# Audio-WestlakeU/FN-SSL

Measured on AMD Instinct MI355X. Metric: TF-frames/sec DP-IPD forward, 4-mic 257-bin x 300-frame, higher is better.
Workload: dtype f32; 1 GPU; BASELINE configs[1]: FN-SSL (online) DP-IPD forward, waveform->STFT->features->3x(full-band BiLSTM + narrow-band LSTM)->head; 32 utterances/GPU x 4 mics ('MM' = 6 pairs) x 257 bins x 300 frames, fp32; frame = one STFT frame of one utterance; stream_chunk_frames=0, utterances_per_gpu=32, global_batch=32, mics=4, pairs_per_utterance=6, frames=300, bins=257, parallelism=dp1 (utterance shards, no collective), chunk_pairs=0

## Files before the change

fn-ssl_amd/csrc/forward.hip:

```cpp
#include <algorithm>

#include "common.h"

namespace {

size_t align_up(size_t v, size_t a) { return (v + a - 1) / a * a; }

struct Plan {
  int chunk;
  size_t act_floats;
  size_t lstm_ws;
  size_t head_floats;
  size_t total;
};

Plan make_plan(int nb, int nf, int nt, int is_online, int chunk_pairs) {
  Plan p;
  p.chunk = (chunk_pairs <= 0 || chunk_pairs > nb) ? nb : chunk_pairs;
  p.act_floats = (size_t)p.chunk * nt * nf * 256;
  const size_t ws_full = fnssl_lstm_workspace_bytes_ex(p.chunk * nt, 128, 2, FNSSL_PRECISION_FP32);
  const size_t ws_narr = is_online ? fnssl_lstm_workspace_bytes_ex(p.chunk * nf, 256, 1, FNSSL_PRECISION_FP32)
                                   : fnssl_lstm_workspace_bytes_ex(p.chunk * nf, 128, 2, FNSSL_PRECISION_FP32);
  p.lstm_ws = align_up(std::max(ws_full, ws_narr), 256);
  p.head_floats = (size_t)p.chunk * (nt / FNSSL_SEG_FRAMES) * 2 * nf;
  p.total = 6 * align_up(p.act_floats * 4, 256) + p.lstm_ws + align_up(p.head_floats * 4, 256) + 256;
  return p;
}

}

extern "C" {

size_t fnssl_forward_workspace_bytes(int nb, int nf, int nt, int is_online, int chunk_pairs) {
  if (nb <= 0 || nf <= 0 || nt <= 0) return 0;
  return make_plan(nb, nf, nt, is_online, chunk_pairs).total;
}

int fnssl_forward(const fnssl_net* net, const float* x0, int nb, int nf, int nt, float* out, void* workspace,
                  size_t workspace_bytes, int chunk_pairs, void* stream) {
  FNSSL_REQUIRE(net && x0, "forward: null pointer");
  FNSSL_REQUIRE(nb > 0 && nf > 0 && nt > 0, "forward: empty problem (nb %d, nf %d, nt %d)", nb, nf, nt);
  if (nt / FNSSL_SEG_FRAMES == 0) return FNSSL_OK;
  FNSSL_REQUIRE(out, "forward: null output pointer");
  FNSSL_REQUIRE(net->input_size > 0 && net->input_size % 4 == 0, "forward: input_size %d must be a multiple of 4",
                net->input_size);
  FNSSL_REQUIRE(!net->doa_wt || nf == 256, "forward: the DOA layer needs nf = 256 (Linear(512, 180))");
  const Plan pl = make_plan(nb, nf, nt, net->is_online, chunk_pairs);
  if (!workspace || workspace_bytes < pl.total) {
    fnssl::set_error("forward: workspace %zu < %zu bytes", workspace_bytes, pl.total);
    return FNSSL_E_WORKSPACE;
  }
  char* wsb = static_cast<char*>(workspace);
  wsb = reinterpret_cast<char*>(align_up(reinterpret_cast<uintptr_t>(wsb), 256));
  const size_t act_bytes = align_up(pl.act_floats * 4, 256);
  float* F[2] = {reinterpret_cast<float*>(wsb), reinterpret_cast<float*>(wsb + act_bytes)};
  float* N[2] = {reinterpret_cast<float*>(wsb + 2 * act_bytes), reinterpret_cast<float*>(wsb + 3 * act_bytes)};
  float* Sf = reinterpret_cast<float*>(wsb + 4 * act_bytes);
  float* Sn = reinterpret_cast<float*>(wsb + 5 * act_bytes);
  float* lws = reinterpret_cast<float*>(wsb + 6 * act_bytes);
  float* head_tmp = reinterpret_cast<float*>(wsb + 6 * act_bytes + pl.lstm_ws);

  const int cin = net->input_size;
  const int nt2 = nt / FNSSL_SEG_FRAMES;
  const int narr_h = net->is_online ? 256 : 128;
  const int narr_dirs = net->is_online ? 1 : 2;
  const long long C = 256;
  const long long PS = (long long)nt * nf * C;
  const fnssl_view fl_by_full = {nullptr, PS, (long long)nf * C, C};
  const fnssl_view fl_by_narr = {nullptr, PS, C, (long long)nf * C};
  const fnssl_view nl_by_full = {nullptr, PS, C, (long long)nt * C};
  const fnssl_view nl_by_narr = {nullptr, PS, (long long)nt * C, C};
  auto with = [](fnssl_view v, const float* p) {
    v.p = p;
    return v;
  };

  for (int p0 = 0; p0 < nb; p0 += pl.chunk) {
    const int G = std::min(pl.chunk, nb - p0);
    const float* xc = x0 + (size_t)p0 * nt * nf * cin;
    for (int blk = 0; blk < 3; ++blk) {
      float* Fo = F[blk & 1];
      float* No = N[blk & 1];
      const float* Np = N[(blk + 1) & 1];
      fnssl_lstm_desc d = {};
      d.hidden = 128;
      d.ndir = 2;
      d.nseq = G * nt;
      d.q_inner = nt;
      d.nsteps = nf;
      if (blk == 0) {
        d.src0 = fnssl_view{xc, (long long)nt * nf * cin, (long long)nf * cin, cin};
        d.c0 = cin;
      } else {
        d.src0 = with(nl_by_full, Sn);
        d.c0 = 256;
      }
      d.out = Fo;
      d.out_so = fl_by_full.so;
      d.out_si = fl_by_full.si;
      d.out_st = fl_by_full.st;
      if (blk > 0) {
        d.skip = with(nl_by_full, Np);
        d.out_sum = Sf;
      }
      d.wpack[0] = net->wpack[blk][0][0];
      d.wpack[1] = net->wpack[blk][0][1];
      d.workspace = lws;
      d.workspace_bytes = pl.lstm_ws;
      d.fallback_count = net->fallback_count;
      d.tuning = net->tuning;
      int rc = fnssl_lstm_forward(&d, stream);
      if (rc != FNSSL_OK) return rc;
      fnssl_lstm_desc e = {};
      e.hidden = narr_h;
      e.ndir = narr_dirs;
      e.nseq = G * nf;
      e.q_inner = nf;
      e.nsteps = nt;
      e.c0 = 256;
      if (blk == 0) {
        e.src0 = with(fl_by_narr, Fo);
        e.src2 = fnssl_view{xc, (long long)nt * nf * cin, cin, (long long)nf * cin};
        e.c2 = cin;
      } else {
        e.src0 = with(fl_by_narr, Sf);
      }
      e.out = No;
      e.out_so = nl_by_narr.so;
      e.out_si = nl_by_narr.si;
      e.out_st = nl_by_narr.st;
      if (blk < 2) {
        e.skip = with(fl_by_narr, Fo);
        e.out_sum = Sn;
      }
      e.wpack[0] = net->wpack[blk][1][0];
      e.wpack[1] = net->wpack[blk][1][1];
      e.workspace = lws;
      e.workspace_bytes = pl.lstm_ws;
      e.fallback_count = net->fallback_count;
      e.tuning = net->tuning;
      rc = fnssl_lstm_forward(&e, stream);
      if (rc != FNSSL_OK) return rc;
    }
    if (nt2 > 0) {
      if (net->doa_wt) {
        int rc = fnssl_head(N[0], G, nf, nt, net->emb_w, net->emb_b, head_tmp, stream);
        if (rc != FNSSL_OK) return rc;
        rc = fnssl_linear(head_tmp, G * nt2, 2 * nf, net->doa_wt, net->doa_b, 180,
                          out + (size_t)p0 * nt2 * 180, stream);
        if (rc != FNSSL_OK) return rc;
      } else {
        int rc = fnssl_head(N[0], G, nf, nt, net->emb_w, net->emb_b, out + (size_t)p0 * nt2 * 2 * nf, stream);
        if (rc != FNSSL_OK) return rc;
      }
    }
  }
  return FNSSL_OK;
}

}
```

fn-ssl_amd/csrc/lstm.hip:

```cpp
#include <algorithm>
#include <cstdlib>
#include <cstring>
#include <vector>

#include "common.h"
#include "tuning.h"

#include "lstm_static.h"
#include "lstm_bf16.h"
#include "lstm_bf16w.h"
#include "lstm_split_static.h"

using namespace fnssl_lstm;

namespace fnssl_lstm {
extern template int launch_h<16>(int, const LstmParams&, int, int, const LaunchCtx&);
extern template int launch_h<32>(int, const LstmParams&, int, int, const LaunchCtx&);
extern template int launch_h<64>(int, const LstmParams&, int, int, const LaunchCtx&);
extern template int launch_h<128>(int, const LstmParams&, int, int, const LaunchCtx&);
extern template int launch_h<256>(int, const LstmParams&, int, int, const LaunchCtx&);
extern template int launch_split_h<128>(int, const LstmParams&, int, int, const LaunchCtx&);
extern template int launch_split_h<256>(int, const LstmParams&, int, int, const LaunchCtx&);
int forward_save(LstmParams p, int H, int mode, const LaunchCtx& lc);
int forward_bf16(LstmParams p, int H, const LaunchCtx& lc);
// ... 232 lines not shown
}

static LstmParams fwd_params(const fnssl_lstm_desc* d, const LstmWsLayout& ws) {
  LstmParams p;
  p.src0 = View{d->src0.p, d->src0.so, d->src0.si, d->src0.st};
  p.src1 = View{d->src1.p, d->src1.so, d->src1.si, d->src1.st};
  p.src2 = View{d->src2.p, d->src2.so, d->src2.si, d->src2.st};
  p.skip = View{d->skip.p, d->skip.so, d->skip.si, d->skip.st};
  p.carry = d->carry_state ? 1 : 0;
  p.out = d->carry_state ? d->out - d->out_st : d->out;
  p.out_sum = (d->carry_state && d->out_sum) ? d->out_sum - d->out_st : d->out_sum;
  p.out_so = d->out_so;
  p.out_si = d->out_si;
  p.out_st = d->out_st;
  p.wpack[0] = d->wpack[0];
  p.wpack[1] = d->wpack[1];
  p.cscratch = d->workspace;
  p.cluster_ws = reinterpret_cast<char*>(d->workspace) + ws.cluster.off;
  p.reserve = d->reserve;
  p.ntasks = (d->nseq + 15) / 16;
  p.c0 = d->c0;
  p.c2 = d->c2;
  p.nseq = d->nseq;
  p.q_inner = d->q_inner;
  p.nsteps = d->nsteps;
  p.ndir = d->ndir;
  p.quads_per_slice = quads_per_slice(d->c0, d->c2, d->hidden);
#ifdef FNSSL_BUILD_ABLATE
  p.ablate = env_int("FNSSL_ABLATE", 1, 255);
#else
  p.ablate = 0;
#endif
  p.fallback_count = d->fallback_count;
  return p;
}

struct Fp32Call {
  const fnssl_lstm_desc* d;
  const LstmWsLayout& ws;
  const LaunchCtx& lc;
  LstmParams p;
  int H, mode;
  int* family;
  int* rounds;
  int nlaunch = 0;
  void report(int f) {
    if (family) *family = f;
  }
  int done(int rc) {
    if (rounds) *rounds = nlaunch;
    return rc;
  }
  int train();
  int inference();
  int planned_rounds();
  int launch_round(int variant, int t0, int t1);
  int launch_round_interleaved_h256(int NW, int nwg);
  int launch_split(int split, bool static_only);
};

int Fp32Call::train() {
  FNSSL_REQUIRE((H == 128 || H == 256) && !(mode & (kHas1 | kSum)),
                "lstm_forward: the reserve-saving forward needs hidden 128/256 and no src1 / out_sum");
  FNSSL_REQUIRE(d->reserve_bytes >= fnssl_lstm_reserve_bytes(d->nseq, H, d->ndir, d->nsteps) && aligned16(d->reserve) &&
                    (long double)d->nsteps * (H / 16) * kReserveRecs * 1024 < 4.0e9L,
                "lstm_forward: reserve buffer too small or misaligned");
// ... 209 lines not shown
```

fn-ssl_amd/csrc/lstm_f32c.h:

```cpp
#pragma once

#include "lstm_static.h"

namespace fnssl_lstm {

constexpr int kF32cWaves = 16;

struct F32ClusterParams {
  unsigned* tags;
  unsigned* status;
  int clusters_per_dir;
  int groups_per_cluster;
  unsigned spin_limit;
  int stall_member;
  int rotate;
  int prio_mode;
};

template <int HH, int NV0, int NS0, int MODE, bool ABLRT = false, int DRIFT = 2, int NW_ = kF32cWaves, int GS = 1>
__global__ void __launch_bounds__(NW_ * 64) lstm_f32c_kernel(const LstmParams p, const F32ClusterParams cp) {
  constexpr int H = HH, NS = H / 16, NW = NW_;
  constexpr int NWS = NW / GS;
  static_assert((GS == 1 || GS == 4) && NW % GS == 0 && (NWS & (NWS - 1)) == 0, "gate split: whole slots, a power of two of them");
  constexpr bool SUM = (MODE & kSum) != 0, SAVE = (MODE & kSave) != 0;
  constexpr bool CAT = (MODE & kHas2) != 0;
  constexpr int QPS = 1 + NV0 + NS0 + NS;
  constexpr int XD = NW_ > 12 ? 4 : 8;
  constexpr bool STRH = H == 256 && GS == 1 && NW_ > 8;
  static_assert((CAT ? NS0 == 1 : !(NV0 && NS0)) && (NV0 == 0 || NV0 % XD == 0) && (H == 128 || H == 256),
                "blocks of src0, or its remainder alone, or blocks of src0 + the remainder quad of src2");
  static_assert(H == 128 || NW_ <= 8 || STRH, "H = 256 with the row of h_{t-1} held: at most two waves per SIMD (register budget)");
  static_assert(!STRH || (NV0 >= XD && (NV0 + NS) % XD == 0), "streamed row: the ring depth divides the block count");
  static_assert(GS == 1 || (!SAVE && !ABLRT), "gate split: inference kernels only");
  extern __shared__ __attribute__((aligned(16))) char smem[];
  const int ABL = ABLRT ? p.ablate : 0;

  const int b = blockIdx.x;
  const int m = (b >> 3) % NS;
  const int cl = ((b >> 3) / NS) * 8 + (b & 7);
  if (cl >= cp.clusters_per_dir * p.ndir) return;
  const int dir = cl / cp.clusters_per_dir;
  const int ck = cl - dir * cp.clusters_per_dir;
  const int g0 = ck * cp.groups_per_cluster;
  const int g1 = g0 + cp.groups_per_cluster < p.ntasks ? g0 + cp.groups_per_cluster : p.ntasks;
  if (__hip_atomic_load(cp.status, __ATOMIC_RELAXED, __HIP_MEMORY_SCOPE_AGENT) != 0) return;
  if (cl == 0 && m == cp.stall_member) return;

  const int lane = threadIdx.x & 63;
  const int n = lane & 15, g = lane >> 4;
  const int w = __builtin_amdgcn_readfirstlane((int)(threadIdx.x >> 6));
  const int ws = GS == 1 ? w : (w >> 2);
  const int gate = GS == 1 ? 0 : (w & 3);
  const bool rev = dir == 1;
  const unsigned vlane = lane * 16;

  {
    const v4f* src = reinterpret_cast<const v4f*>(reinterpret_cast<const char*>(p.wpack[dir]) + (size_t)(m * QPS) * 4096);
    v4f* dst = reinterpret_cast<v4f*>(smem);
    for (int i = threadIdx.x; i < QPS * 4 * 64; i += NW * 64) dst[i] = src[i];
  }
  char* const xch = smem + QPS * 4096;
  unsigned* const xcnt = reinterpret_cast<unsigned*>(xch + NWS * 2 * 4 * 1024);
  if (GS > 1 && threadIdx.x < NWS) xcnt[threadIdx.x] = 0;
  __syncthreads();
  const char* const lds_rd = smem + lane * 16;
  auto rec = [&](int q, int j) { return *reinterpret_cast<const v4f*>(lds_rd + (q * 4 + j) * 1024); };
  auto rec1 = [&](int q, int j) { return *reinterpret_cast<const float*>(lds_rd + (q * 4 + j) * 1024 + 4 * gate); };

  const unsigned st0 = (unsigned)(p.src0.st * 4), sto = (unsigned)(p.out_st * 4), stk = SUM ? (unsigned)(p.skip.st * 4) : 0u;
  const unsigned st2 = CAT ? (unsigned)(p.src2.st * 4) : 0u;
  const unsigned cy = (unsigned)p.carry;
  unsigned* const tag_cl = cp.tags + (size_t)cl * cp.groups_per_cluster * NS;
  const v4f zero4 = v4f{0.f, 0.f, 0.f, 0.f};

  unsigned pub_val = 0;
  unsigned* pub_tag = nullptr;
  auto pub_flush = [&]() {
    if (pub_tag) {
      asm volatile("s_waitcnt vmcnt(0)" ::: "memory");
      if (lane == 0) __hip_atomic_store(pub_tag, pub_val, __ATOMIC_RELAXED, __HIP_MEMORY_SCOPE_AGENT);
      pub_tag = nullptr;
    }
  };

  struct Grp {
    unsigned vo0, voo, vok, voo2, vo2 = 0;
    bool valid;
    int task, step;
  };
  auto locate = [&](int task, int qo0, int qi0, Grp& gr, rsrc_t& rx0, rsrc_t& ro, rsrc_t& rsk, rsrc_t& ro2, rsrc_t& rx2) {
    const int q0 = task * 16;
    gr.valid = q0 + n < p.nseq;
    const int d = q0 + n < p.nseq ? n : p.nseq - 1 - q0;
    const bool crossed = qi0 + d >= p.q_inner;
    auto one = [&](const float* base, long long so, long long si, int extra, unsigned& voff) {
      const long long delta = (long long)d * si + (crossed ? so - (long long)p.q_inner * si : 0ll);
      voff = (unsigned)(delta * 4) + (unsigned)(extra * 4);
      return make_rsrc(base + ((long long)qo0 * so + (long long)qi0 * si));
    };
    rx0 = one(p.src0.p, p.src0.so, p.src0.si, (NS0 && !CAT) ? g : 4 * g, gr.vo0);
    if constexpr (CAT) rx2 = one(p.src2.p, p.src2.so, p.src2.si, g, gr.vo2);
    ro = one(p.out, p.out_so, p.out_si, dir * H + 4 * g, gr.voo);
    gr.vok = gr.voo2 = 0;
    rsk = SUM ? one(p.skip.p, p.skip.so, p.skip.si, dir * H + 4 * g, gr.vok) : rx0;
    ro2 = SUM ? one(p.out_sum, p.out_so, p.out_si, dir * H + 4 * g, gr.voo2) : ro;
  };
  auto tt_of = [&](int step) { return (unsigned)(rev ? p.nsteps - 1 - step : step); };
  auto rc_of = [&](int task) {
    return make_rsrc(cell_record<NS>(p.cscratch, p.ntasks, dir, task));
  };

  if (g0 + ws >= g1) return;
  unsigned long long clk0 = 0, rt0 = 0;
  if (ABLRT && (ABL & 512)) {
    clk0 = __builtin_amdgcn_s_memtime();
    rt0 = __builtin_amdgcn_s_memrealtime();
  }
  bool dead = false;
  auto bounded_wait = [&](auto ready, auto reload, int sleep, unsigned code) {
    for (unsigned spins = 0; !ready(); ++spins) {
      if (GS > 1) __builtin_amdgcn_s_sleep(1); else if (sleep == 8) __builtin_amdgcn_s_sleep(8); else __builtin_amdgcn_s_sleep(16);
      reload();
      const bool out = spins > cp.spin_limit;
      if (out || (spins & 63) == 63) {
        if (out) {
          if (lane == 0) __hip_atomic_store(cp.status, code | (unsigned)(cl & 0xffff), __ATOMIC_RELAXED, __HIP_MEMORY_SCOPE_AGENT);
          return false;
        }
        if (__hip_atomic_load(cp.status, __ATOMIC_RELAXED, __HIP_MEMORY_SCOPE_AGENT) != 0) return false;
      }
    }
    return true;
  };
  const int NGR = g1 - g0;
  const bool rot = cp.rotate && NGR >= 2 * NWS;
  const int FULL = rot ? (NGR / NWS) * NWS : NGR, LEFT = NGR - FULL;
  const bool single = GS == 1 && g0 + ws + NWS >= g1;
  Grp cur, nxt;
  rsrc_t rx0, ro, rsk, ro2, rx2, nrx0, nro, nrsk, nro2, nrx2;
  v4f xr[XD];
  float xs0 = 0.f;
  v4f cprev = zero4, skipv = zero4;
  unsigned tagv = 0, tagd = 0;
  auto request = [&](const Grp& gr, rsrc_t qx0, rsrc_t qsk, bool with_c, bool with_x = true) {
    const unsigned tt = tt_of(gr.step);
    if (!(ABL & 8)) {
      if constexpr (NV0 > 0) if (with_x) static_for<XD>([&](auto v) { xr[v.value] = bld4(qx0, gr.vo0, tt * st0 + 64 * v.value); });
      if constexpr (NS0 > 0 && !CAT) xs0 = bld1(qx0, gr.vo0, tt * st0);
    }
    if (SUM && !(ABL & 64)) skipv = bld4(qsk, gr.vok, tt * stk + 64 * m);
    if (gr.step > 0 || cy) {
      if (gr.step > 0 && !(ABL & 256))
        tagv = __hip_atomic_load(tag_cl + (size_t)(gr.task - g0) * NS + (lane & (NS - 1)), __ATOMIC_RELAXED, __HIP_MEMORY_SCOPE_AGENT);
      if (GS == 1 && with_c && !(ABL & 64)) cprev = bld4_l2(rc_of(gr.task), vlane, m * 1024);
    }
    if (DRIFT > 0 && !(ABL & 256) && gr.task - DRIFT * NWS >= g0)
      tagd = __hip_atomic_load(tag_cl + (size_t)(gr.task - DRIFT * NWS - g0) * NS + (lane & (NS - 1)), __ATOMIC_RELAXED, __HIP_MEMORY_SCOPE_AGENT);
  };
  cur.task = g0 + ws;
  cur.step = 0;
  unsigned iter = 0;
  const int qo_first = (cur.task * 16) / p.q_inner, qi_first = cur.task * 16 - qo_first * p.q_inner;
  int qo0 = qo_first, qi0 = qi_first;
  locate(cur.task, qo0, qi0, cur, rx0, ro, rsk, ro2, rx2);
  request(cur, rx0, rsk, true);
  if constexpr (CAT) xs0 = bld1(rx2, cur.vo2, tt_of(0) * st2);

  for (;;) {
    const int step = cur.step, task = cur.task;
    const unsigned tt = tt_of(step);
    const unsigned o0 = tt * st0, oo = (tt + cy) * sto;
    const unsigned op = (rev ? tt + 1 : tt - 1 + cy) * sto;
    const rsrc_t rc = rc_of(task);
    unsigned* const tag_g = tag_cl + (size_t)(task - g0) * NS;
    if (single && (step > 0 || cy) && !(ABL & 64)) cprev = bld4_l2(rc, vlane, m * 1024);
    const bool late_c = GS > 1 || task >= g0 + FULL;
    v4f cprev_cur = (step > 0 || cy) ? cprev : zero4;
    const v4f skip_cur = skipv;

    v4f hold[STRH ? 1 : NS];
    auto fetch_h = [&]() {
      if (DRIFT > 0 && !(ABL & 4) && !dead && task - DRIFT * NWS >= g0) {
        unsigned* const tag_d = tag_cl + (size_t)(task - DRIFT * NWS - g0) * NS;
        dead = !bounded_wait([&]() { return __builtin_amdgcn_ballot_w64(tagd < (unsigned)step + 1) == 0; },
                             [&]() { tagd = __hip_atomic_load(tag_d + (lane & (NS - 1)), __ATOMIC_RELAXED, __HIP_MEMORY_SCOPE_AGENT); }, 8, 0x40000u);
      }
      if ((step > 0 || cy) && !(ABL & 16)) {
        if (step > 0 && !(ABL & 4) && !dead)
          dead = !bounded_wait([&]() { return __builtin_amdgcn_ballot_w64(tagv < (unsigned)step) == 0; },
                               [&]() { tagv = __hip_atomic_load(tag_g + (lane & (NS - 1)), __ATOMIC_RELAXED, __HIP_MEMORY_SCOPE_AGENT); }, 16, 0x30000u);
        if (late_c && !(ABL & 64)) cprev_cur = bld4_l2(rc, vlane, m * 1024);
        if constexpr (!STRH) {
#pragma unroll
          for (int s = 0; s < NS; ++s) hold[s] = bld4_l2(ro, cur.voo, op + 64 * s);
        }
      } else if constexpr (!STRH) {
#pragma unroll
        for (int s = 0; s < NS; ++s) hold[s] = (ABL & 16) ? cprev : zero4;
      }
    };
    const bool hrow = step > 0 || cy;
    auto hblock = [&](int j) { return hrow ? bld4_l2(ro, cur.voo, op + 64 * j) : zero4; };

    if (cp.prio_mode == 2) __builtin_amdgcn_s_setprio(2);
    v4f acc[4];
    v4f ra[4];
    v4f acc1 = zero4;
    float rb[4] = {0.f, 0.f, 0.f, 0.f};
    if constexpr (GS == 1) {
      acc[0] = rec(0, 0);
      acc[1] = rec(0, 1);
// ... 18 lines not shown
        return;
      }
      MFMA4(acc, ra[0], b0);
      __builtin_amdgcn_sched_barrier(0);
      if constexpr (Q + 1 < QPS) if (!(ABL & 128)) ra[0] = rec(Q + 1, 0);
      __builtin_amdgcn_sched_barrier(0);
      MFMA4(acc, ra[1], b1);
      __builtin_amdgcn_sched_barrier(0);
      if constexpr (Q + 1 < QPS) if (!(ABL & 128)) ra[1] = rec(Q + 1, 1);
      __builtin_amdgcn_sched_barrier(0);
      MFMA4(acc, ra[2], b2);
      __builtin_amdgcn_sched_barrier(0);
      if constexpr (Q + 1 < QPS) if (!(ABL & 128)) ra[2] = rec(Q + 1, 2);
      __builtin_amdgcn_sched_barrier(0);
      MFMA4(acc, ra[3], b3);
      __builtin_amdgcn_sched_barrier(0);
      if constexpr (Q + 1 < QPS) if (!(ABL & 128)) ra[3] = rec(Q + 1, 3);
      __builtin_amdgcn_sched_barrier(0);
    };
    auto quad1 = [&](auto qc, float b0) {
      constexpr int Q = decltype(qc)::value;
      if constexpr (GS > 1) {
        acc1 = __builtin_amdgcn_mfma_f32_16x16x4f32(rb[0], b0, acc1, 0, 0, 0);
        if constexpr (Q + 1 < QPS) static_for<4>([&](auto j) { rb[j.value] = rec1(Q + 1, j.value); });
        return;
      }
      MFMA4(acc, ra[0], b0);
      if constexpr (Q + 1 < QPS) static_for<4>([&](auto j) { ra[j.value] = rec(Q + 1, j.value); });
    };
    if constexpr (NV0 > 0) {
      static_for<NV0>([&](auto v) {
        constexpr int V = decltype(v)::value;
        if constexpr (STRH) {
          if constexpr (V == NV0 / 2) pub_flush();
          if constexpr (V == NV0 - XD) fetch_h();
        } else if constexpr (V == NV0 / 2) {
          pub_flush();
          fetch_h();
        }
        const v4f xb = xr[V % XD];
        quad(ic<1 + V>{}, xb.x, xb.y, xb.z, xb.w);
        if constexpr (V + XD < NV0) {
          if (!(ABL & 8)) xr[V % XD] = bld4(rx0, cur.vo0, o0 + 64 * (V + XD));
        } else if constexpr (STRH) {
          xr[V % XD] = hblock(V + XD - NV0);
        }
      });
      if constexpr (NS0 > 0) quad1(ic<1 + NV0>{}, xs0);
    } else {
      pub_flush();
      fetch_h();
      quad1(ic<1>{}, xs0);
    }
    bool seq_next = false;
    if (task < g0 + FULL && task + NWS < g0 + FULL) {
      nxt.task = task + NWS;
      nxt.step = step;
      seq_next = true;
    } else {
      const int j = (ws - step) & (NWS - 1);
      if (task < g0 + FULL && j < LEFT) {
        nxt.task = g0 + FULL + j;
        nxt.step = step;
      } else {
        nxt.task = g0 + ws;
        nxt.step = step + 1;
      }
// ... 5 lines not shown
        nrx0 = rx0; nro = ro; nrsk = rsk; nro2 = ro2;
        if constexpr (CAT) {
          nxt.vo2 = cur.vo2;
          nrx2 = rx2;
        }
      } else {
        if (seq_next) {
          qi0 += 16 * NWS;
          while (qi0 >= p.q_inner) {
            qi0 -= p.q_inner;
            ++qo0;
          }
        } else if (nxt.step == step) {
          qo0 = (nxt.task * 16) / p.q_inner;
          qi0 = nxt.task * 16 - qo0 * p.q_inner;
        } else {
          qo0 = qo_first;
          qi0 = qi_first;
        }
        locate(nxt.task, qo0, qi0, nxt, nrx0, nro, nrsk, nro2, nrx2);
      }
      request(nxt, nrx0, nrsk, !single && nxt.task < g0 + FULL, !STRH);
      if constexpr (CAT) xs0 = bld1(nrx2, nxt.vo2, tt_of(nxt.step) * st2);
    }
    static_for<NS>([&](auto sp) {
      constexpr int SP = decltype(sp)::value;
      if constexpr (STRH) {
        constexpr int B = NV0 + SP, B2 = B + XD;
        const v4f hb = xr[B % XD];
        quad(ic<1 + NV0 + NS0 + SP>{}, hb.x, hb.y, hb.z, hb.w);
        if constexpr (B2 < NV0 + NS) {
          xr[B % XD] = hblock(B2 - NV0);
        } else {
          if (more) xr[B % XD] = bld4(nrx0, nxt.vo0, tt_of(nxt.step) * st0 + 64 * (B2 - NV0 - NS));
        }
      } else {
        quad(ic<1 + NV0 + NS0 + SP>{}, hold[SP].x, hold[SP].y, hold[SP].z, hold[SP].w);
      }
    });

    if (cp.prio_mode == 2) __builtin_amdgcn_s_setprio(0);
    if (dead) break;
    v4f cn, hn;
    if (ABL & 2) {
      cn = acc[1] + cprev_cur + acc[0];
      hn = acc[3] + acc[2];
    } else {
      v4f ig, fg, gg, og;
      if constexpr (GS == 1) {
        ig = sigmoid4(acc[0]);
        fg = sigmoid4(acc[1]);
        gg = tanh4(acc[2]);
        og = sigmoid4(acc[3]);
      } else {
        const v4f act = gate == 2 ? tanh4(acc1) : sigmoid4(acc1);
        v4f* const xb = reinterpret_cast<v4f*>(xch + (size_t)((ws * 2 + (int)(iter & 1u)) * 4) * 1024);
        xb[gate * 64 + lane] = act;
        asm volatile("s_waitcnt lgkmcnt(0)" ::: "memory");
        if (lane == 0) __hip_atomic_fetch_add(xcnt + ws, 1u, __ATOMIC_RELAXED, __HIP_MEMORY_SCOPE_WORKGROUP);
        const unsigned want = 4u * (iter + 1u);
        for (unsigned spins = 0;; ++spins) {
          if (__hip_atomic_load(xcnt + ws, __ATOMIC_RELAXED, __HIP_MEMORY_SCOPE_WORKGROUP) >= want) break;
          if (dead || ((spins & 63u) == 63u && __hip_atomic_load(cp.status, __ATOMIC_RELAXED, __HIP_MEMORY_SCOPE_AGENT) != 0u) ||
              spins > cp.spin_limit) {
            dead = true;
            break;
          }
          __builtin_amdgcn_s_sleep(1);
        }
        asm volatile("" ::: "memory");
        ig = xb[lane];
        fg = xb[64 + lane];
        gg = xb[128 + lane];
        og = xb[192 + lane];
        ++iter;
      }
      cn = cell4(fg, cprev_cur, ig, gg);
      hn = mul_rn4(og, tanh4(cn));
      if constexpr (SAVE) {
        const rsrc_t rres = make_rsrc(reinterpret_cast<const char*>(p.reserve) +
                                      ((size_t)dir * p.ntasks + task) * p.nsteps * (size_t)(NS * kReserveRecs * 1024));
        const unsigned rb = (tt * NS + m) * (kReserveRecs * 1024);
        bst4(ig, rres, vlane, rb);
        bst4(fg, rres, vlane, rb + 1024);
        bst4(gg, rres, vlane, rb + 2048);
        bst4(og, rres, vlane, rb + 3072);
        bst4(cn, rres, vlane, rb + 4096);
      }
    }
    asm("" : "+v"(hn.x), "+v"(hn.y), "+v"(hn.z), "+v"(hn.w));
    if (ABL & 32) asm volatile("" ::"v"(cn), "v"(hn));
    const bool storer = GS == 1 || gate == 0;
    if (storer && !(ABL & 32)) bst4(cn, rc, vlane, m * 1024);
    if (storer && cur.valid && !(ABL & 32)) {
      __builtin_amdgcn_raw_buffer_store_b128(__builtin_bit_cast(v4u, hn), ro, cur.voo, oo + 64 * m, 16);
      if (SUM) bst4(add_rn4(hn, skip_cur), ro2, cur.voo2, oo + 64 * m);
    }
    pub_val = __builtin_amdgcn_readfirstlane((unsigned)step + 1);
    pub_tag = ((ABL & 256) || !storer) ? nullptr : tag_g + m;
    if (GS > 1 || single) pub_flush();
    if (!more || dead) break;
    cur = nxt;
    rx0 = nrx0;
    ro = nro;
    rsk = nrsk;
    ro2 = nro2;
    if constexpr (CAT) rx2 = nrx2;
  }
  pub_flush();
  asm volatile("s_waitcnt vmcnt(0)" ::: "memory");
  if (ABLRT && (ABL & 512) && (w == 0 || w == 15) && lane == 0) {
    const unsigned long long c1 = __builtin_amdgcn_s_memtime(), r1 = __builtin_amdgcn_s_memrealtime();
    printf("f32c blk %d wave %d start %llu end %llu cycles %llu MHz %.1f\n", b, w, rt0, r1, c1 - clk0,
           (double)(c1 - clk0) / (double)(r1 - rt0) * 100.0);
  }
}

template <int HH, int NV0, int NS0, int MODE, bool ABLRT = false, int DRIFT = 2, int NW_ = kF32cWaves, int GS = 1>
int launch_f32c_k(const LstmParams& p, const F32ClusterParams& cp, const LaunchCtx& lc) {
  constexpr int NS = HH / 16;
  constexpr int QPS = 1 + NV0 + NS0 + NS;
  const size_t lds = (size_t)QPS * 4096 + (GS > 1 ? (size_t)(NW_ / GS) * 8192 + 64 : 0);
  static_assert(QPS * 4096 + (GS > 1 ? (NW_ / GS) * 8192 + 64 : 0) <= 160 * 1024, "LDS");
  const int ncl = cp.clusters_per_dir * p.ndir;
  const int nwg = 8 * NS * ((ncl + 7) / 8);
  return enqueue(lc, Kernel{lstm_f32c_kernel<HH, NV0, NS0, MODE, ABLRT, DRIFT, NW_, GS>, NW_ * 64, lds, "lstm_f32c_kernel", true}, nwg, p, cp);
}

}
// ... 1 lines not shown
```

fn-ssl_amd/csrc/lstm_f32c.hip:

```cpp
#include <cstdlib>

#include "lstm_f32c.h"
#include "tuning.h"

namespace fnssl_lstm {

constexpr int kF32cWavesH256 = 16;
constexpr int kF32cWavesH256Split = 8;

static bool f32c_uniform(const LstmParams& p, int mode) {
  auto even = [&](long long so, long long si) { return si >= 0 && so == (long long)p.q_inner * si; };
  return even(p.src0.so, p.src0.si) && even(p.out_so, p.out_si) && (!(mode & kSum) || even(p.skip.so, p.skip.si)) &&
         (!(mode & kHas2) || even(p.src2.so, p.src2.si));
}

bool f32c_handles(const LstmParams& p, int H, int mode) {
  if (fnssl::tune(FNSSL_TUNE_NO_F32_CLUSTER)) return false;
  if ((H != 128 && H != 256) || p.ablate) return false;
  if (H == 128) {
    if (p.c2 != 0 || p.carry) return false;
    if (p.reserve && mode != 0) return false;
    if (!(p.c0 == 256 && (mode == kSum || mode == 0)) && !(p.c0 == 4 && mode == 0 && !fnssl::tune(FNSSL_TUNE_NO_F32C_B1))) return false;
  } else {
    if (p.ndir != 1 || p.c0 != 256 || fnssl::tune(FNSSL_TUNE_NO_F32_SMALL)) return false;
    const bool plain = p.c2 == 0 && (mode == 0 || mode == kSum), cat = p.c2 == 4 && (mode == kHas2 || mode == (kHas2 | kSum));
    if (!plain && !cat) return false;
    if (p.reserve && ((mode & kSum) || p.carry)) return false;
  }
  auto grows = [&](long long so, long long si) { return si >= 0 && so >= (long long)(p.q_inner - 1) * si; };
  if (!f32c_uniform(p, mode) &&
      (p.q_inner < 16 || !grows(p.src0.so, p.src0.si) || !grows(p.out_so, p.out_si) ||
       ((mode & kSum) && !grows(p.skip.so, p.skip.si)) || ((mode & kHas2) && !grows(p.src2.so, p.src2.si))))
    return false;
  const int ncu = cluster_cus();
  if (ncu < (H / 16) * p.ndir) return false;
  const long long groups = (long long)p.ntasks * p.ndir;
  if (const int mg = fnssl::tune(FNSSL_TUNE_F32C_MIN_GROUPS, 1, 1 << 30)) {
    if (groups < mg) return false;
  }
  if (p.reserve) {
    if (fnssl::tune(FNSSL_TUNE_TRAIN_NO_F32_CLUSTER)) return false;
    return true;
  }
  if (H == 256) {
    const long long full = 12LL * ncu, rounds = (groups + full - 1) / full;
    return groups < full || groups * 100 < rounds * full * 97;
  }
  return !fnssl::tune(FNSSL_TUNE_NO_F32_SMALL) || groups >= 12LL * ncu;
}

template <int NW_, int GS>
static int launch_f32c_h256(const LstmParams& p, const F32ClusterParams& cp, int mode, const LaunchCtx& lc) {
  if (mode == (kHas2 | kSum)) return launch_f32c_k<256, 16, 1, kHas2 | kSum, false, 2, NW_, GS>(p, cp, lc);
  if (mode == kHas2) return launch_f32c_k<256, 16, 1, kHas2, false, 2, NW_, GS>(p, cp, lc);
  if (mode == kSum) return launch_f32c_k<256, 16, 0, kSum, false, 2, NW_, GS>(p, cp, lc);
  return launch_f32c_k<256, 16, 0, 0, false, 2, NW_, GS>(p, cp, lc);
}

int forward_f32c(LstmParams p, int H, int mode, size_t cluster_bytes, const LaunchCtx& lc) {
  if (f32c_uniform(p, mode)) p.q_inner = p.nseq;
  const int ncu = cluster_cus();
  const int members = H / 16;
  F32ClusterParams cp;
  cp.clusters_per_dir = (ncu / members) / p.ndir;
  cp.groups_per_cluster = (p.ntasks + cp.clusters_per_dir - 1) / cp.clusters_per_dir;
  cp.status = reinterpret_cast<unsigned*>(p.cluster_ws);
  cp.tags = reinterpret_cast<unsigned*>(p.cluster_ws + 256);
  cp.spin_limit = cluster_spin_limit();
  cp.stall_member = cluster_test_stall();
  cp.rotate = !fnssl::tune(FNSSL_TUNE_F32C_NO_ROTATE);
  cp.prio_mode = fnssl::tune(FNSSL_TUNE_F32C_PRIO, 9, 9) ? 0 : 2;
  const size_t tag_bytes = (size_t)p.ndir * cp.clusters_per_dir * cp.groups_per_cluster * members * sizeof(unsigned);
  FNSSL_REQUIRE(256 + tag_bytes <= cluster_bytes, "lstm_forward: the cluster kernel's tags exceed the workspace's cluster area");
  if (!lc.dry) FNSSL_HIP(hipMemsetAsync(p.cluster_ws, 0, 256 + tag_bytes, lc.st));
  const int gs_knob = fnssl::tune(FNSSL_TUNE_F32C_GATE_SPLIT, 1, 4);
  const bool gsplit = gs_knob ? gs_knob == 4 : cp.groups_per_cluster <= 1;
  if (H == 256) {
    constexpr int W = kF32cWavesH256;
    if (p.reserve)
      return p.c2 == 4 ? launch_f32c_k<256, 16, 1, kHas2 | kSave, false, 2, W>(p, cp, lc) : launch_f32c_k<256, 16, 0, kSave, false, 2, W>(p, cp, lc);
    if (gsplit) return launch_f32c_h256<kF32cWavesH256Split, 4>(p, cp, mode, lc);
    if (cp.groups_per_cluster <= kF32cWavesH256Split) return launch_f32c_h256<kF32cWavesH256Split, 1>(p, cp, mode, lc);
    return launch_f32c_h256<W, 1>(p, cp, mode, lc);
  }
  if (gsplit && !p.reserve) {
    if (p.c0 == 4) return launch_f32c_k<128, 0, 1, 0, false, 2, kF32cWaves, 4>(p, cp, lc);
    if (mode == kSum) return launch_f32c_k<128, 16, 0, kSum, false, 2, kF32cWaves, 4>(p, cp, lc);
    return launch_f32c_k<128, 16, 0, 0, false, 2, kF32cWaves, 4>(p, cp, lc);
  }
#ifdef FNSSL_BUILD_ABLATE
  if (const int abl = env_int("FNSSL_F32C_ABL", 1, 1023)) {
    p.ablate = abl;
    if (mode == kSum) return launch_f32c_k<128, 16, 0, kSum, true>(p, cp, lc);
    if (p.c0 == 4) return launch_f32c_k<128, 0, 1, 0, true>(p, cp, lc);
  }
  p.ablate = 0;
#endif
  if (p.reserve) return p.c0 == 4 ? launch_f32c_k<128, 0, 1, kSave>(p, cp, lc) : launch_f32c_k<128, 16, 0, kSave>(p, cp, lc);
  if (p.c0 == 4) return launch_f32c_k<128, 0, 1, 0>(p, cp, lc);
  if (mode == kSum) return launch_f32c_k<128, 16, 0, kSum>(p, cp, lc);
  return launch_f32c_k<128, 16, 0, 0>(p, cp, lc);
}

}
```

fn-ssl_amd/csrc/lstm_host.h:

```cpp
#pragma once

#include "host.h"
#include "tuning.h"

namespace fnssl_lstm {

constexpr int kNoStatic = -100;
constexpr int kNoCluster = -101;

using fnssl::aligned16;
using fnssl::check_workspace;
using fnssl::enqueue;
using fnssl::Kernel;
using fnssl::LaunchCtx;
using fnssl::WsRegion;

inline unsigned cluster_spin_limit() {
  const int v = fnssl::tune(FNSSL_TUNE_CLUSTER_SPIN_LIMIT, 1, 1 << 30);
  return v ? (unsigned)v : (1u << 20);
}
inline int cluster_test_stall() { return fnssl::tune(FNSSL_TUNE_CLUSTER_TEST_STALL, 1, 1 << 20) - 1; }
inline int cluster_cus() {
  const int ncu = fnssl::device_cus();
  int r = fnssl::tune(FNSSL_TUNE_RESERVED_CUS, 1, ncu);
  r = (r + 7) / 8 * 8;
  return r >= ncu ? 0 : ncu - r;
}
template <class C, class F>
int cluster_then_fallback(const LaunchCtx& lc, bool handles, int cluster_family, int* family, const void* status, C&& cluster,
                          F&& fallback) {
  const unsigned* guard = nullptr;
  if (handles) {
    const int rc = cluster();
    if (rc == FNSSL_OK) {
      if (family) *family = cluster_family;
      if (lc.dry) return FNSSL_OK;
      guard = static_cast<const unsigned*>(status);
    } else if (rc != kNoCluster) {
      return rc;
    }
  }
  return fallback(guard);
}

inline bool mult4(long long so, long long si, long long st) { return ((so | si | st) & 3) == 0; }
inline bool mult4(const fnssl_view& v) { return mult4(v.so, v.si, v.st); }
inline bool nonneg(long long so, long long si, long long st) { return so >= 0 && si >= 0 && st >= 0; }
inline bool extent_ok(long long so, long long si, long long st, long long width, int nsteps) {
  return nonneg(so, si, st) && ((long double)so + 16.0L * si + (long double)nsteps * st + width) * 4.0L < 4.0e9L;
}
inline bool extent_ok(const fnssl_view& v, long long width, int nsteps) { return extent_ok(v.so, v.si, v.st, width, nsteps); }

}
```

fn-ssl_amd/csrc/lstm_kernel.h:

```cpp
#pragma once

#include <cstdio>
#include <cstdlib>
#include <type_traits>

#include "common.h"
#include "tuning.h"
#include "lstm_host.h"

#pragma clang fp contract(off)

typedef float v4f __attribute__((ext_vector_type(4)));

namespace fnssl_lstm {

struct View {
  const float* p;
  long long so, si, st;
};

struct LstmParams {
  View src0, src1, src2, skip;
  float* out;
  float* out_sum;
  long long out_so, out_si, out_st;
  const float* wpack[2];
  float* cscratch;
  char* cluster_ws;
  float* reserve;
  int ntasks;
  int carry;
  int c0, c2;
  int nseq, q_inner, nsteps, ndir;
  int wgs_per_dir;
  int task0, task1;
  int quads_per_slice;
  int chq, pad;
  int ablate;
  const unsigned* guard = nullptr;
  unsigned* fallback_count = nullptr;
};

#define FNSSL_GUARDED_KERNEL(P)                                                                            \
  do {                                                                                                     \
    if ((P).guard) {                                                                                       \
      if (__hip_atomic_load((P).guard, __ATOMIC_RELAXED, __HIP_MEMORY_SCOPE_AGENT) == 0) return;           \
      if ((P).fallback_count && blockIdx.x == 0 && threadIdx.x == 0 && (P).task0 == 0) atomicAdd((P).fallback_count, 1u); \
    }                                                                                                      \
  } while (0)

__host__ __device__ constexpr int cluster_members(int H) { return H == 256 ? 8 : 4; }
__host__ __device__ constexpr int cluster_parts(int H) { return H == 256 ? 2 : 3; }
__host__ __device__ constexpr int cluster_seqs(int H) { return cluster_parts(H) * 256; }
__host__ __device__ constexpr size_t cluster_parity_bytes(int H) {
  return (size_t)cluster_parts(H) * 8 * (H / 16) * 1024;
}
constexpr int kClusterTagWords = 256;

constexpr int kHas1 = 1;
constexpr int kHas2 = 2;
constexpr int kSum = 4;
constexpr int kSave = 8;

constexpr int kSpareTasks = 16;
template <int NS>
__device__ __forceinline__ const char* cell_record(const float* cscratch, int ntasks, int dir, int slot) {
  return reinterpret_cast<const char*>(cscratch) + ((size_t)dir * (ntasks + kSpareTasks) + slot) * (NS * 1024);
}
template <int NS>
__device__ __forceinline__ const char* dhdc_record(const float* scratch, int ntasks, int dir, int slot) {
  return reinterpret_cast<const char*>(scratch) + ((size_t)dir * (ntasks + kSpareTasks) + slot) * (2 * NS * 1024);
}

constexpr int kReserveRecs = 5;

__host__ __device__ inline int quads_per_slice(int c0, int c2, int H) {
  return 1 + (c0 >> 4) + ((c0 & 15) >> 2) + (c2 >> 4) + ((c2 & 15) >> 2) + (H >> 4);
}

__device__ __forceinline__ float sigmoid_f(float x) {
  return __builtin_amdgcn_rcpf(__fadd_rn(1.0f, __expf(-x)));
}
__device__ __forceinline__ float tanh_f(float x) {
  return __fmaf_rn(-2.0f, __builtin_amdgcn_rcpf(__fadd_rn(__expf(2.0f * x), 1.0f)), 1.0f);
}
typedef float v2f __attribute__((ext_vector_type(2)));
__device__ __forceinline__ v2f exp2_2(v2f a) { return v2f{__builtin_amdgcn_exp2f(a.x), __builtin_amdgcn_exp2f(a.y)}; }
__device__ __forceinline__ v2f rcp_2(v2f a) { return v2f{__builtin_amdgcn_rcpf(a.x), __builtin_amdgcn_rcpf(a.y)}; }
__device__ __forceinline__ v2f sigmoid2(v2f a) {
  const v2f nl2e = {-0x1.715476p+0f, -0x1.715476p+0f};
  const v2f one = {1.0f, 1.0f};
  return rcp_2(exp2_2(a * nl2e) + one);
}
__device__ __forceinline__ v2f tanh2(v2f a) {
  const v2f l2e2 = {0x1.715476p+1f, 0x1.715476p+1f};
// ... 566 lines not shown
```

fn-ssl_amd/csrc/tuning.h:

```cpp
#pragma once

#include "../../include/fnssl.h"

namespace fnssl {

const fnssl_tuning& tuning();

inline int tune(int index) { return tuning().knob[index]; }
inline int tune(int index, int lo, int hi) {
  const int v = tune(index);
  return v >= lo && v <= hi ? v : 0;
}

struct TuningScope {
  explicit TuningScope(const fnssl_tuning* t);
  ~TuningScope();
  TuningScope(const TuningScope&) = delete;
  TuningScope& operator=(const TuningScope&) = delete;
  const fnssl_tuning* prev_;
  bool active_;
};

}
```

Measured before the change: 18080 frames/s.

## Interleave activation and residual-sum slabs so LSTM reads skip via paired buffer offsets

The forward pass now lays out each LSTM output next to its residual-sum buffer, and each input next to its skip tensor, in one slab with a doubled pair stride. The f32c cluster kernel gains a paired mode in which the skip value and the sum output are reached through a fixed byte delta from the existing src0 and out buffer resources. This removes two separate buffer descriptors and their per-step address math. The skip load is also moved into the middle of the compute loop so it overlaps other work. The trade-off is more template instantiations, larger strides with possibly worse locality per tensor, and added offset-range checks, with a tuning knob to switch the mode off.

```diff
diff --git a/fn-ssl_amd/csrc/forward.hip b/fn-ssl_amd/csrc/forward.hip
--- a/fn-ssl_amd/csrc/forward.hip
+++ b/fn-ssl_amd/csrc/forward.hip
@@ -53,10 +53,15 @@
   char* wsb = static_cast<char*>(workspace);
   wsb = reinterpret_cast<char*>(align_up(reinterpret_cast<uintptr_t>(wsb), 256));
   const size_t act_bytes = align_up(pl.act_floats * 4, 256);
-  float* F[2] = {reinterpret_cast<float*>(wsb), reinterpret_cast<float*>(wsb + act_bytes)};
-  float* N[2] = {reinterpret_cast<float*>(wsb + 2 * act_bytes), reinterpret_cast<float*>(wsb + 3 * act_bytes)};
-  float* Sf = reinterpret_cast<float*>(wsb + 4 * act_bytes);
-  float* Sn = reinterpret_cast<float*>(wsb + 5 * act_bytes);
+  const long long C = 256;
+  const long long PS = (long long)nt * nf * C;
+  const bool slabs = nt >= 16;
+  const long long SO = slabs ? 2 * PS : PS;
+  float* F[2] = {reinterpret_cast<float*>(wsb), slabs ? reinterpret_cast<float*>(wsb) : reinterpret_cast<float*>(wsb + act_bytes)};
+  float* Sf = slabs ? F[0] + PS : reinterpret_cast<float*>(wsb + 4 * act_bytes);
+  float* Sn = reinterpret_cast<float*>(wsb + (slabs ? 2 : 5) * act_bytes);
+  float* N[2] = {slabs ? Sn + PS : reinterpret_cast<float*>(wsb + 2 * act_bytes), slabs ? Sn + PS : reinterpret_cast<float*>(wsb + 3 * act_bytes)};
+  float* Nlast = slabs ? reinterpret_cast<float*>(wsb + 4 * act_bytes) : N[0];
   float* lws = reinterpret_cast<float*>(wsb + 6 * act_bytes);
   float* head_tmp = reinterpret_cast<float*>(wsb + 6 * act_bytes + pl.lstm_ws);
 
@@ -64,12 +69,10 @@
   const int nt2 = nt / FNSSL_SEG_FRAMES;
   const int narr_h = net->is_online ? 256 : 128;
   const int narr_dirs = net->is_online ? 1 : 2;
-  const long long C = 256;
-  const long long PS = (long long)nt * nf * C;
-  const fnssl_view fl_by_full = {nullptr, PS, (long long)nf * C, C};
-  const fnssl_view fl_by_narr = {nullptr, PS, C, (long long)nf * C};
-  const fnssl_view nl_by_full = {nullptr, PS, C, (long long)nt * C};
-  const fnssl_view nl_by_narr = {nullptr, PS, (long long)nt * C, C};
+  const fnssl_view fl_by_full = {nullptr, SO, (long long)nf * C, C};
+  const fnssl_view fl_by_narr = {nullptr, SO, C, (long long)nf * C};
+  const fnssl_view nl_by_full = {nullptr, SO, C, (long long)nt * C};
+  const fnssl_view nl_by_narr = {nullptr, SO, (long long)nt * C, C};
   auto with = [](fnssl_view v, const float* p) {
     v.p = p;
     return v;
@@ -80,7 +83,7 @@
     const float* xc = x0 + (size_t)p0 * nt * nf * cin;
     for (int blk = 0; blk < 3; ++blk) {
       float* Fo = F[blk & 1];
-      float* No = N[blk & 1];
+      float* No = blk == 2 ? Nlast : N[blk & 1];
       const float* Np = N[(blk + 1) & 1];
       fnssl_lstm_desc d = {};
       d.hidden = 128;
@@ -126,7 +129,7 @@
         e.src0 = with(fl_by_narr, Sf);
       }
       e.out = No;
-      e.out_so = nl_by_narr.so;
+      e.out_so = blk == 2 ? PS : nl_by_narr.so;
       e.out_si = nl_by_narr.si;
       e.out_st = nl_by_narr.st;
       if (blk < 2) {
@@ -144,13 +147,13 @@
     }
     if (nt2 > 0) {
       if (net->doa_wt) {
-        int rc = fnssl_head(N[0], G, nf, nt, net->emb_w, net->emb_b, head_tmp, stream);
+        int rc = fnssl_head(Nlast, G, nf, nt, net->emb_w, net->emb_b, head_tmp, stream);
         if (rc != FNSSL_OK) return rc;
         rc = fnssl_linear(head_tmp, G * nt2, 2 * nf, net->doa_wt, net->doa_b, 180,
                           out + (size_t)p0 * nt2 * 180, stream);
         if (rc != FNSSL_OK) return rc;
       } else {
-        int rc = fnssl_head(N[0], G, nf, nt, net->emb_w, net->emb_b, out + (size_t)p0 * nt2 * 2 * nf, stream);
+        int rc = fnssl_head(Nlast, G, nf, nt, net->emb_w, net->emb_b, out + (size_t)p0 * nt2 * 2 * nf, stream);
         if (rc != FNSSL_OK) return rc;
       }
     }
diff --git a/fn-ssl_amd/csrc/lstm.hip b/fn-ssl_amd/csrc/lstm.hip
--- a/fn-ssl_amd/csrc/lstm.hip
+++ b/fn-ssl_amd/csrc/lstm.hip
@@ -288,6 +288,9 @@
   p.ablate = 0;
 #endif
   p.fallback_count = d->fallback_count;
+  if (d->out_sum && !fnssl::tune(FNSSL_TUNE_NO_PAIRED_SUM))
+    residual_pair(d->src0, d->skip, d->out, d->out_sum, d->out_so, d->out_si, d->out_st, 2 * d->hidden, d->nsteps, d->carry_state != 0,
+                  &p.skip_delta, &p.sum_delta);
   return p;
 }
 
diff --git a/fn-ssl_amd/csrc/lstm_f32c.h b/fn-ssl_amd/csrc/lstm_f32c.h
--- a/fn-ssl_amd/csrc/lstm_f32c.h
+++ b/fn-ssl_amd/csrc/lstm_f32c.h
@@ -23,6 +23,8 @@
   constexpr int NWS = NW / GS;
   static_assert((GS == 1 || GS == 4) && NW % GS == 0 && (NWS & (NWS - 1)) == 0, "gate split: whole slots, a power of two of them");
   constexpr bool SUM = (MODE & kSum) != 0, SAVE = (MODE & kSave) != 0;
+  constexpr bool PAIR = (MODE & kPaired) != 0;
+  static_assert(!PAIR || (SUM && NV0 > 0), "paired: a fused residual on 16-channel input blocks");
   constexpr bool CAT = (MODE & kHas2) != 0;
   constexpr int QPS = 1 + NV0 + NS0 + NS;
   constexpr int XD = NW_ > 12 ? 4 : 8;
@@ -67,7 +69,11 @@
   auto rec = [&](int q, int j) { return *reinterpret_cast<const v4f*>(lds_rd + (q * 4 + j) * 1024); };
   auto rec1 = [&](int q, int j) { return *reinterpret_cast<const float*>(lds_rd + (q * 4 + j) * 1024 + 4 * gate); };
 
-  const unsigned st0 = (unsigned)(p.src0.st * 4), sto = (unsigned)(p.out_st * 4), stk = SUM ? (unsigned)(p.skip.st * 4) : 0u;
+  const unsigned st0 = (unsigned)(p.src0.st * 4), sto = (unsigned)(p.out_st * 4), stk = (SUM && !PAIR) ? (unsigned)(p.skip.st * 4) : 0u;
+  const unsigned xadd = (PAIR && p.skip_delta < 0) ? (unsigned)-p.skip_delta : 0u;
+  const unsigned kadd = (PAIR && p.skip_delta > 0 ? (unsigned)p.skip_delta : 0u) + (unsigned)(dir * H * 4 + 64 * m);
+  const unsigned oadd = (PAIR && p.sum_delta < 0) ? (unsigned)-p.sum_delta : 0u;
+  const unsigned sadd = (PAIR && p.sum_delta > 0 ? (unsigned)p.sum_delta : 0u) + (unsigned)(64 * m);
   const unsigned st2 = CAT ? (unsigned)(p.src2.st * 4) : 0u;
   const unsigned cy = (unsigned)p.carry;
   unsigned* const tag_cl = cp.tags + (size_t)cl * cp.groups_per_cluster * NS;
@@ -98,12 +104,12 @@
       voff = (unsigned)(delta * 4) + (unsigned)(extra * 4);
       return make_rsrc(base + ((long long)qo0 * so + (long long)qi0 * si));
     };
-    rx0 = one(p.src0.p, p.src0.so, p.src0.si, (NS0 && !CAT) ? g : 4 * g, gr.vo0);
+    rx0 = one(PAIR ? reinterpret_cast<const float*>(reinterpret_cast<const char*>(p.src0.p) - xadd) : p.src0.p, p.src0.so, p.src0.si, (NS0 && !CAT) ? g : 4 * g, gr.vo0);
     if constexpr (CAT) rx2 = one(p.src2.p, p.src2.so, p.src2.si, g, gr.vo2);
-    ro = one(p.out, p.out_so, p.out_si, dir * H + 4 * g, gr.voo);
+    ro = one(PAIR ? reinterpret_cast<const float*>(reinterpret_cast<const char*>(p.out) - oadd) : p.out, p.out_so, p.out_si, dir * H + 4 * g, gr.voo);
     gr.vok = gr.voo2 = 0;
-    rsk = SUM ? one(p.skip.p, p.skip.so, p.skip.si, dir * H + 4 * g, gr.vok) : rx0;
-    ro2 = SUM ? one(p.out_sum, p.out_so, p.out_si, dir * H + 4 * g, gr.voo2) : ro;
+    rsk = (SUM && !PAIR) ? one(p.skip.p, p.skip.so, p.skip.si, dir * H + 4 * g, gr.vok) : rx0;
+    ro2 = (SUM && !PAIR) ? one(p.out_sum, p.out_so, p.out_si, dir * H + 4 * g, gr.voo2) : ro;
   };
   auto tt_of = [&](int step) { return (unsigned)(rev ? p.nsteps - 1 - step : step); };
   auto rc_of = [&](int task) {
@@ -145,10 +151,10 @@
   auto request = [&](const Grp& gr, rsrc_t qx0, rsrc_t qsk, bool with_c, bool with_x = true) {
     const unsigned tt = tt_of(gr.step);
     if (!(ABL & 8)) {
-      if constexpr (NV0 > 0) if (with_x) static_for<XD>([&](auto v) { xr[v.value] = bld4(qx0, gr.vo0, tt * st0 + 64 * v.value); });
-      if constexpr (NS0 > 0 && !CAT) xs0 = bld1(qx0, gr.vo0, tt * st0);
-    }
-    if (SUM && !(ABL & 64)) skipv = bld4(qsk, gr.vok, tt * stk + 64 * m);
+      if constexpr (NV0 > 0) if (with_x) static_for<XD>([&](auto v) { xr[v.value] = bld4(qx0, gr.vo0, tt * st0 + xadd + 64 * v.value); });
+      if constexpr (NS0 > 0 && !CAT) xs0 = bld1(qx0, gr.vo0, tt * st0 + xadd);
+    }
+    if (SUM && !PAIR && !(ABL & 64)) skipv = bld4(qsk, gr.vok, tt * stk + 64 * m);
     if (gr.step > 0 || cy) {
       if (gr.step > 0 && !(ABL & 256))
         tagv = __hip_atomic_load(tag_cl + (size_t)(gr.task - g0) * NS + (lane & (NS - 1)), __ATOMIC_RELAXED, __HIP_MEMORY_SCOPE_AGENT);
@@ -169,14 +175,17 @@
   for (;;) {
     const int step = cur.step, task = cur.task;
     const unsigned tt = tt_of(step);
-    const unsigned o0 = tt * st0, oo = (tt + cy) * sto;
-    const unsigned op = (rev ? tt + 1 : tt - 1 + cy) * sto;
+    const unsigned o0 = tt * st0 + xadd, oo = (tt + cy) * sto + oadd;
+    const unsigned op = (rev ? tt + 1 : tt - 1 + cy) * sto + oadd;
     const rsrc_t rc = rc_of(task);
     unsigned* const tag_g = tag_cl + (size_t)(task - g0) * NS;
     if (single && (step > 0 || cy) && !(ABL & 64)) cprev = bld4_l2(rc, vlane, m * 1024);
     const bool late_c = GS > 1 || task >= g0 + FULL;
     v4f cprev_cur = (step > 0 || cy) ? cprev : zero4;
-    const v4f skip_cur = skipv;
+    v4f skip_cur = skipv;
+    auto fetch_skip = [&]() {
+      if constexpr (PAIR) if (!(ABL & 64)) skip_cur = bld4(rx0, cur.vo0, tt * st0 + kadd);
+    };
 
     v4f hold[STRH ? 1 : NS];
     auto fetch_h = [&]() {
@@ -261,7 +270,10 @@
       static_for<NV0>([&](auto v) {
         constexpr int V = decltype(v)::value;
         if constexpr (STRH) {
-          if constexpr (V == NV0 / 2) pub_flush();
+          if constexpr (V == NV0 / 2) {
+            pub_flush();
+            fetch_skip();
+          }
           if constexpr (V == NV0 - XD) fetch_h();
         } else if constexpr (V == NV0 / 2) {
           pub_flush();
@@ -333,9 +345,10 @@
         if constexpr (B2 < NV0 + NS) {
           xr[B % XD] = hblock(B2 - NV0);
         } else {
-          if (more) xr[B % XD] = bld4(nrx0, nxt.vo0, tt_of(nxt.step) * st0 + 64 * (B2 - NV0 - NS));
+          if (more) xr[B % XD] = bld4(nrx0, nxt.vo0, tt_of(nxt.step) * st0 + xadd + 64 * (B2 - NV0 - NS));
         }
       } else {
+        if constexpr (SP == 1) fetch_skip();
         quad(ic<1 + NV0 + NS0 + SP>{}, hold[SP].x, hold[SP].y, hold[SP].z, hold[SP].w);
       }
     });
@@ -395,7 +408,8 @@
     if (storer && !(ABL & 32)) bst4(cn, rc, vlane, m * 1024);
     if (storer && cur.valid && !(ABL & 32)) {
       __builtin_amdgcn_raw_buffer_store_b128(__builtin_bit_cast(v4u, hn), ro, cur.voo, oo + 64 * m, 16);
-      if (SUM) bst4(add_rn4(hn, skip_cur), ro2, cur.voo2, oo + 64 * m);
+      if constexpr (PAIR) bst4(add_rn4(hn, skip_cur), ro, cur.voo, (tt + cy) * sto + sadd);
+      else if (SUM) bst4(add_rn4(hn, skip_cur), ro2, cur.voo2, oo + 64 * m);
     }
     pub_val = __builtin_amdgcn_readfirstlane((unsigned)step + 1);
     pub_tag = ((ABL & 256) || !storer) ? nullptr : tag_g + m;
diff --git a/fn-ssl_amd/csrc/lstm_f32c.hip b/fn-ssl_amd/csrc/lstm_f32c.hip
--- a/fn-ssl_amd/csrc/lstm_f32c.hip
+++ b/fn-ssl_amd/csrc/lstm_f32c.hip
@@ -51,6 +51,8 @@
 
 template <int NW_, int GS>
 static int launch_f32c_h256(const LstmParams& p, const F32ClusterParams& cp, int mode, const LaunchCtx& lc) {
+  if (mode == (kHas2 | kSum | kPaired)) return launch_f32c_k<256, 16, 1, kHas2 | kSum | kPaired, false, 2, NW_, GS>(p, cp, lc);
+  if (mode == (kSum | kPaired)) return launch_f32c_k<256, 16, 0, kSum | kPaired, false, 2, NW_, GS>(p, cp, lc);
   if (mode == (kHas2 | kSum)) return launch_f32c_k<256, 16, 1, kHas2 | kSum, false, 2, NW_, GS>(p, cp, lc);
   if (mode == kHas2) return launch_f32c_k<256, 16, 1, kHas2, false, 2, NW_, GS>(p, cp, lc);
   if (mode == kSum) return launch_f32c_k<256, 16, 0, kSum, false, 2, NW_, GS>(p, cp, lc);
@@ -59,6 +61,8 @@
 
 int forward_f32c(LstmParams p, int H, int mode, size_t cluster_bytes, const LaunchCtx& lc) {
   if (f32c_uniform(p, mode)) p.q_inner = p.nseq;
+  const bool paired = (mode & kSum) && p.skip_delta != 0 && p.sum_delta != 0;
+  const int kmode = paired ? (mode | kPaired) : mode;
   const int ncu = cluster_cus();
   const int members = H / 16;
   F32ClusterParams cp;
@@ -79,18 +83,20 @@
     constexpr int W = kF32cWavesH256;
     if (p.reserve)
       return p.c2 == 4 ? launch_f32c_k<256, 16, 1, kHas2 | kSave, false, 2, W>(p, cp, lc) : launch_f32c_k<256, 16, 0, kSave, false, 2, W>(p, cp, lc);
-    if (gsplit) return launch_f32c_h256<kF32cWavesH256Split, 4>(p, cp, mode, lc);
-    if (cp.groups_per_cluster <= kF32cWavesH256Split) return launch_f32c_h256<kF32cWavesH256Split, 1>(p, cp, mode, lc);
-    return launch_f32c_h256<W, 1>(p, cp, mode, lc);
+    if (gsplit) return launch_f32c_h256<kF32cWavesH256Split, 4>(p, cp, kmode, lc);
+    if (cp.groups_per_cluster <= kF32cWavesH256Split) return launch_f32c_h256<kF32cWavesH256Split, 1>(p, cp, kmode, lc);
+    return launch_f32c_h256<W, 1>(p, cp, kmode, lc);
   }
   if (gsplit && !p.reserve) {
     if (p.c0 == 4) return launch_f32c_k<128, 0, 1, 0, false, 2, kF32cWaves, 4>(p, cp, lc);
+    if (paired) return launch_f32c_k<128, 16, 0, kSum | kPaired, false, 2, kF32cWaves, 4>(p, cp, lc);
     if (mode == kSum) return launch_f32c_k<128, 16, 0, kSum, false, 2, kF32cWaves, 4>(p, cp, lc);
     return launch_f32c_k<128, 16, 0, 0, false, 2, kF32cWaves, 4>(p, cp, lc);
   }
 #ifdef FNSSL_BUILD_ABLATE
   if (const int abl = env_int("FNSSL_F32C_ABL", 1, 1023)) {
     p.ablate = abl;
+    if (paired) return launch_f32c_k<128, 16, 0, kSum | kPaired, true>(p, cp, lc);
     if (mode == kSum) return launch_f32c_k<128, 16, 0, kSum, true>(p, cp, lc);
     if (p.c0 == 4) return launch_f32c_k<128, 0, 1, 0, true>(p, cp, lc);
   }
@@ -98,6 +104,7 @@
 #endif
   if (p.reserve) return p.c0 == 4 ? launch_f32c_k<128, 0, 1, kSave>(p, cp, lc) : launch_f32c_k<128, 16, 0, kSave>(p, cp, lc);
   if (p.c0 == 4) return launch_f32c_k<128, 0, 1, 0>(p, cp, lc);
+  if (paired) return launch_f32c_k<128, 16, 0, kSum | kPaired>(p, cp, lc);
   if (mode == kSum) return launch_f32c_k<128, 16, 0, kSum>(p, cp, lc);
   return launch_f32c_k<128, 16, 0, 0>(p, cp, lc);
 }
diff --git a/fn-ssl_amd/csrc/lstm_host.h b/fn-ssl_amd/csrc/lstm_host.h
--- a/fn-ssl_amd/csrc/lstm_host.h
+++ b/fn-ssl_amd/csrc/lstm_host.h
@@ -51,4 +51,27 @@
 }
 inline bool extent_ok(const fnssl_view& v, long long width, int nsteps) { return extent_ok(v.so, v.si, v.st, width, nsteps); }
 
+inline bool pair_distance_ok(long long delta_bytes, long long so, long long si, long long st, long long width, long long rows) {
+  const long long dist = delta_bytes < 0 ? -delta_bytes : delta_bytes;
+  if (dist == 0 || (dist & 15) || !nonneg(so, si, st)) return false;
+  const long double reach = ((long double)so + 16.0L * si + (long double)rows * st + width) * 4.0L;
+  return reach + (long double)dist < 2147483648.0L;
 }
+inline long long byte_distance(const void* a, const void* b) {
+  return (long long)(reinterpret_cast<intptr_t>(b) - reinterpret_cast<intptr_t>(a));
+}
+inline bool residual_pair(const fnssl_view& src0, const fnssl_view& skip, const float* out, const float* out_sum, long long out_so,
+                          long long out_si, long long out_st, int width, int nsteps, bool carry, int* skip_delta, int* sum_delta) {
+  *skip_delta = *sum_delta = 0;
+  if (!src0.p || !skip.p || !out || !out_sum) return false;
+  if (skip.so != src0.so || skip.si != src0.si || skip.st != src0.st) return false;
+  const long long dk = byte_distance(src0.p, skip.p), ds = byte_distance(out, out_sum);
+  if (!pair_distance_ok(dk, src0.so, src0.si, src0.st, width, nsteps) ||
+      !pair_distance_ok(ds, out_so, out_si, out_st, width, (long long)nsteps + (carry ? 1 : 0)))
+    return false;
+  *skip_delta = (int)dk;
+  *sum_delta = (int)ds;
+  return true;
+}
+
+}
diff --git a/fn-ssl_amd/csrc/lstm_kernel.h b/fn-ssl_amd/csrc/lstm_kernel.h
--- a/fn-ssl_amd/csrc/lstm_kernel.h
+++ b/fn-ssl_amd/csrc/lstm_kernel.h
@@ -39,6 +39,8 @@
   int ablate;
   const unsigned* guard = nullptr;
   unsigned* fallback_count = nullptr;
+  int skip_delta = 0, sum_delta = 0;
+  int pair_pad_[2] = {0, 0};
 };
 
 #define FNSSL_GUARDED_KERNEL(P)                                                                            \
@@ -61,6 +63,7 @@
 constexpr int kHas2 = 2;
 constexpr int kSum = 4;
 constexpr int kSave = 8;
+constexpr int kPaired = 16;
 
 constexpr int kSpareTasks = 16;
 template <int NS>
diff --git a/fn-ssl_amd/csrc/tuning.h b/fn-ssl_amd/csrc/tuning.h
--- a/fn-ssl_amd/csrc/tuning.h
+++ b/fn-ssl_amd/csrc/tuning.h
@@ -1,6 +1,9 @@
 #pragma once
 
 #include "../../include/fnssl.h"
+
+#define FNSSL_TUNE_NO_PAIRED_SUM 42
+static_assert(FNSSL_TUNE_NO_PAIRED_SUM < FNSSL_TUNE_COUNT, "knob index beyond fnssl_tuning");
 
 namespace fnssl {
 
```

New measurement: 18170 frames/s, median of 6. Within noise of the previous version (+0.5%).
